# noegroup/aggforce

Hardware: AMD Instinct MI355X
Metric: frames/sec through project_forces (Gram+solve), 1e6x4096-atom traj, 1/2/4/8 GPU (higher is better)
Workload: dtype f64

## Files before the change

aggforce_amd/csrc/aggf_gram.hip:

```cpp
#include <stdlib.h>

#include "aggf_common.h"
#include "aggf_routing.h"

#include <type_traits>

namespace aggf {

constexpr int TILE = 128;
constexpr int ROW_ELEMS = TILE * 3;
constexpr int ROW_PAD = 16;
constexpr int ROW_STRIDE = ROW_ELEMS + ROW_PAD;

template <typename T>
struct GramCfg;
template <>
struct GramCfg<double> {
  static constexpr int KB = 4;
};
template <>
struct GramCfg<float> {
  static constexpr int KB = 8;
};

// ... 269 lines not shown
  if (AHEAD > 1 && n_it > 1) issue_stage(1);
  if (AHEAD > 1 && n_it > 1 && ragged_seq != 1) {
    if constexpr (EDGE) wait_vmcnt_dyn<8>(n_act); else wait_vmcnt<PPW>();
  } else {
    wait_vmcnt<0>();
  }
  asm volatile("s_waitcnt lgkmcnt(0)" ::: "memory");
  __builtin_amdgcn_s_barrier();
  asm volatile("" ::: "memory");

#ifdef AGGF_GRAM_PROF
  uint64_t prof_issue = 0, prof_compute = 0, prof_sync = 0;
#endif
  for (int it = 0; it < n_it; ++it) {
    AGGF_PROF_T(p0);
    constexpr int GROUPS = 3 * KB / 4;
    constexpr bool SPREAD = SPREAD_DMA;
    const bool issue_now = (ABL == 0 || ABL >= 3) && it + AHEAD < n_it;
    if (issue_now) {
      if (SPREAD) prep_stage(it + AHEAD); else issue_stage(it + AHEAD);
    }
    const TS* pa = smem + (((ABL == 1 || ABL == 2) ? it % 2 : it % NBUF)) * BUF_ELEMS;
    AGGF_PROF_T(p1);
    T aL[ES > 0 ? ES : 1][4], bL[ES > 0 ? ES : 1][NACC];
    (void)aL;
    (void)bL;
#pragma unroll
    for (int kk = 0; kk < KB / 4; ++kk) {
#pragma unroll
      for (int d = 0; d < 3; ++d) {
        constexpr int ESG = EARLY_SYNC ? ES : 0;
        const int g = kk * 3 + d;
        T a[4], bb[NACC];
        if (ESG > 0 && g == GROUPS - ESG) {
#pragma unroll
          for (int h = 0; h < (ESG > 0 ? ESG : 1); ++h) {
            const int kh = (GROUPS - ESG + h) / 3, dh = (GROUPS - ESG + h) % 3;
#pragma unroll
            for (int m = 0; m < 4; ++m) aL[h][m] = (T)pa[offA + kh * KKS + 48 * m + dh];
#pragma unroll
            for (int n = 0; n < NACC; ++n) bL[h][n] = (T)pa[offB + kh * KKS + 48 * n + dh];
          }
        }
        if (ESG > 0 && g >= GROUPS - ESG) {
#pragma unroll
          for (int m = 0; m < 4; ++m) a[m] = aL[g - (GROUPS - ESG)][m];
#pragma unroll
          for (int n = 0; n < NACC; ++n) bb[n] = bL[g - (GROUPS - ESG)][n];
        } else {
#pragma unroll
          for (int m = 0; m < 4; ++m) a[m] = (T)pa[offA + kk * KKS + 48 * m + d];
#pragma unroll
          for (int n = 0; n < NACC; ++n) bb[n] = (T)pa[offB + kk * KKS + 48 * n + d];
        }
        constexpr bool DMA_AFTER = ES_DMA_AFTER && ESG > 0;
        if (SPREAD && issue_now && !(DMA_AFTER && g == GROUPS - ESG)) {
#pragma unroll
          for (int q = 0; q < PPW; ++q)
            if (dma_piece_group(GROUPS, PPW, q) == g) issue_piece(it + AHEAD, q);
        }
        if (ESG > 0 && g == GROUPS - ESG) {
          constexpr int ISSUED = dma_pieces_upto(GROUPS, PPW, GROUPS - ESG - (DMA_AFTER ? 1 : 0));
          static_assert(ISSUED >= 0 && ISSUED <= PPW, "pieces issued by the barrier group");
          if (AHEAD > 1 && it + 2 < n_it && it + 2 != ragged_seq) {
            if constexpr (EDGE) wait_vmcnt_dyn<8>(n_act_early); else wait_vmcnt<ISSUED>();
          } else {
            wait_vmcnt<0>();
          }
          asm volatile("s_waitcnt lgkmcnt(0)" ::: "memory");
          __builtin_amdgcn_s_barrier();
          asm volatile("" ::: "memory");
          if (DMA_AFTER && SPREAD && issue_now) {
#pragma unroll
            for (int q = 0; q < PPW; ++q)
              if (dma_piece_group(GROUPS, PPW, q) == g) issue_piece(it + AHEAD, q);
          }
        }
#pragma unroll
        for (int m = 0; m < 4; ++m)
#pragma unroll
          for (int n = 0; n < NACC; ++n) acc[m][n] = M::mma(a[m], bb[n], acc[m][n]);
      }
    }
    AGGF_PROF_T(p2);
    if (ABL != 2 && !EARLY_SYNC) {
      if (AHEAD > 1 && it + 2 < n_it && it + 2 != ragged_seq) {
        if constexpr (EDGE) wait_vmcnt_dyn<8>(n_act); else wait_vmcnt<PPW>();
      } else {
        wait_vmcnt<0>();
      }
      asm volatile("s_waitcnt lgkmcnt(0)" ::: "memory");
      __builtin_amdgcn_s_barrier();
      asm volatile("" ::: "memory");
    }
#ifdef AGGF_GRAM_PROF
    const uint64_t p3 = __builtin_readcyclecounter();
    prof_issue += p1 - p0;
    prof_compute += p2 - p1;
    prof_sync += p3 - p2;
#endif
  }
#ifdef AGGF_GRAM_PROF
  if (lane == 0) {
    atomicAdd(&aggf_gram_prof[0], (unsigned long long)prof_issue);
    atomicAdd(&aggf_gram_prof[1], (unsigned long long)prof_compute);
    atomicAdd(&aggf_gram_prof[2], (unsigned long long)prof_sync);
    atomicAdd(&aggf_gram_prof[3], (unsigned long long)n_it);
  }
#endif

  T* slab = slabs + ((int64_t)tile_lin * ksplit + ks) * (TILE * TILE);
#pragma unroll
  for (int m = 0; m < 4; ++m)
#pragma unroll
    for (int n = 0; n < NACC; ++n)
#pragma unroll
      for (int r = 0; r < 4; ++r) {
        const int row = wm * 64 + m * 16 + M::row(lane, r);
        const int col = wn * WCOLS + n * 16 + (lane & 15);
        slab[row * TILE + col] = acc[m][n][r];
      }
}

__global__ __launch_bounds__(256) void build_tile_table_kernel(int32_t nt1, int32_t* __restrict__ table,
                                                              int32_t first_tile = 0) {
  __shared__ int wave_count[4];
  const int lane = threadIdx.x & 63, wave = threadIdx.x >> 6;
  const int64_t nsb = (nt1 + 7) / 8, n_super = nsb * (nsb + 1) / 2;
  int64_t base = 0;
  for (int64_t b0 = 0; b0 < n_super; b0 += 4) {
    const int64_t sb = b0 + wave;
    bool keep = false;
    int ti = 0, tj = 0;
    if (sb < n_super) {
      const double w = 2.0 * (double)nsb + 1.0;
      int64_t si = (int64_t)((w - sqrt(w * w - 8.0 * (double)sb)) * 0.5);
      if (si < 0) si = 0;
      if (si >= nsb) si = nsb - 1;
      while (si > 0 && si * nsb - si * (si - 1) / 2 > sb) --si;
      while (si + 1 < nsb && (si + 1) * nsb - (si + 1) * si / 2 <= sb) ++si;
      const int64_t sj = si + (sb - (si * nsb - si * (si - 1) / 2));
      ti = (int)si * 8 + (lane >> 3);
      tj = (int)sj * 8 + (lane & 7);
      keep = ti < nt1 && tj < nt1 && tj >= ti && tj >= first_tile;
    }
    const unsigned long long mask = __ballot(keep);
    if (lane == 0) wave_count[wave] = __popcll(mask);
    __syncthreads();
    int64_t off = base;
    for (int w2 = 0; w2 < wave; ++w2) off += wave_count[w2];
    if (keep) table[off + __popcll(mask & ((1ull << lane) - 1ull))] = (ti << 16) | tj;
    base += wave_count[0] + wave_count[1] + wave_count[2] + wave_count[3];
    __syncthreads();
  }
}

template <typename T>
__global__ __launch_bounds__(256) void gram_reduce_kernel(const T* __restrict__ slabs,
                                                          int32_t nt1, int32_t ksplit,
                                                          int32_t n_red, int accumulate,
                                                          double* __restrict__ G, int32_t first_tile = 0) {
  AGGF_GATED_BODY_BEGIN
  int tile = blockIdx.x;
  const int tile_lin = tile;
  int ti = 0;
  {
    int rowlen = nt1;
    while (tile >= rowlen) {
      tile -= rowlen;
      --rowlen;
      ++ti;
    }
  }
  const int tj = ti + tile;
  if (tj < first_tile) return;
  const T* base = slabs + (int64_t)tile_lin * ksplit * (TILE * TILE);
  const int r0 = blockIdx.y * 8;
  for (int e = threadIdx.x; e < 8 * TILE; e += blockDim.x) {
    const int row = r0 + e / TILE, col = e % TILE;
    double s = 0.0;
    for (int ks = 0; ks < ksplit; ++ks)
      s += (double)base[(int64_t)ks * (TILE * TILE) + row * TILE + col];
    const int gi = ti * TILE + row, gj = tj * TILE + col;
    if (gi < n_red && gj < n_red) {
      if (ti != tj || gj >= gi) {
        double* p = G + (int64_t)gi * n_red + gj;
        *p = accumulate ? *p + s : s;
      }
      if (ti != tj || gj > gi) {
        double* p = G + (int64_t)gj * n_red + gi;
        *p = accumulate ? *p + s : s;
      }
    }
  }
  AGGF_GATED_BODY_END
}

constexpr int SM_MAXVEC = 8;
constexpr int SM_FAST_MEMBERS = 4;

template <typename TIn>
static size_t small_raw_bytes(int32_t N, int kbs) { return (size_t)round_up((int64_t)kbs * 3 * N * sizeof(TIn), 16) + 16; }

template <typename TIn, typename TC, int NV, int KBS, int NWV, int W, int C>
__global__ __launch_bounds__(64 * NWV, NWV == 4 ? 3 : 4) void gram_small_kernel(
    const TIn* __restrict__ F, int64_t T, int32_t N, const int32_t* __restrict__ grp_ptr,
    const int32_t* __restrict__ grp_atoms, int32_t n_red, int64_t frames_per_split, int32_t raw_bytes,
    TC* __restrict__ slabs) {
  using M = Mfma<TC>;
  using acc_t = typename M::acc_t;
  constexpr int SM_THREADS = 64 * NWV;
  constexpr int RE = 3 * W, RS = RE + ROW_PAD;
  constexpr int WT = W > TILE ? W : TILE;
  constexpr int SM_ENT = KBS * RE / SM_THREADS;
  constexpr int SM_MAXBLK = C;
  static_assert(KBS * RE % SM_THREADS == 0 && KBS >= 4 && (KBS * W == 8 * TILE || (KBS == 4 && W > 2 * TILE) || (KBS == 8 && W == 2 * TILE)), "entry split");
  typedef float __attribute__((ext_vector_type(4))) v16_t;
  typedef float __attribute__((ext_vector_type(4), aligned(4))) v16g_t;
  extern __shared__ __attribute__((aligned(16))) char smem_raw[];
  TC* panel = reinterpret_cast<TC*>(smem_raw);
  TIn* raw = reinterpret_cast<TIn*>(smem_raw + KBS * RS * sizeof(TC));
  int32_t* atoms_s = reinterpret_cast<int32_t*>(smem_raw + KBS * RS * sizeof(TC) + raw_bytes);
  int32_t* ptr_s = atoms_s + N;
  unsigned short* memb_s = reinterpret_cast<unsigned short*>(smem_raw + KBS * RS * sizeof(TC) + raw_bytes +
                                                             (((int64_t)N + WT + 1) * 4 + 15) / 16 * 16);
  const int tid = threadIdx.x, lane = tid & 63;
  const int wave = __builtin_amdgcn_readfirstlane(tid >> 6);
  (void)frames_per_split;
  const int64_t n_stage_all = (T + KBS - 1) / KBS;
  const int n_it = blockIdx.x < n_stage_all ? (int)((n_stage_all - 1 - blockIdx.x) / gridDim.x + 1) : 0;
  const int64_t t_end = T;
  auto stage_t0 = [&](int k) { return ((int64_t)blockIdx.x + (int64_t)k * gridDim.x) * KBS; };
  const int64_t row_in = (int64_t)N * 3;
  for (int a = tid; a < N; a += SM_THREADS) atoms_s[a] = grp_atoms ? grp_atoms[a] : a;
  for (int g = tid; g <= WT; g += SM_THREADS) ptr_s[g] = g <= n_red ? (grp_ptr ? grp_ptr[g] : g) : (grp_ptr ? grp_ptr[n_red] : n_red);
  const int zero_idx = (raw_bytes - 16) / (int)sizeof(TIn);
  if (tid < 16 / (int)sizeof(TIn)) raw[zero_idx + tid] = (TIn)0;
  __syncthreads();
  bool big_groups = false;
  bool pair_groups = true;
  for (int g = 0; g < n_red; ++g) {
    big_groups |= ptr_s[g + 1] - ptr_s[g] > SM_FAST_MEMBERS;
    pair_groups &= ptr_s[g + 1] - ptr_s[g] <= 2;
  }
  for (int c = tid; c < RE; c += SM_THREADS) {
    const int g = c / 3, d = c - 3 * g;
#pragma unroll
    for (int j = 0; j < SM_FAST_MEMBERS; ++j)
      memb_s[c * 4 + j] = (ptr_s[g] + j < ptr_s[g + 1]) ? (unsigned short)(3 * atoms_s[ptr_s[g] + j] + d) : (unsigned short)0xFFFF;
  }

  const int n_vec = raw_bytes / 16 - 1;
  v16_t hold[NV];
  auto fetch = [&](int s) {
    const int64_t t0 = stage_t0(s);
    const int64_t valid = (t_end - t0 < KBS ? t_end - t0 : KBS) * row_in * (int64_t)sizeof(TIn);
    const char* src = reinterpret_cast<const char*>(F + t0 * row_in);
    if (valid >= (int64_t)n_vec * 16) {
      const unsigned voff = (unsigned)tid * 16u;
      if (gridDim.y == 1) {
#pragma unroll
        for (int i = 0; i < NV; ++i) {
          const int v = tid + SM_THREADS * i;
          const char* base_i = src + (int64_t)i * (SM_THREADS * 16);
          v16_t x = {0.f, 0.f, 0.f, 0.f};
          if (v < n_vec) x = __builtin_nontemporal_load(reinterpret_cast<const v16g_t*>(base_i + voff));
          hold[i] = x;
        }
      } else {
#pragma unroll
        for (int i = 0; i < NV; ++i) {
          const int v = tid + SM_THREADS * i;
          const char* base_i = src + (int64_t)i * (SM_THREADS * 16);
          v16_t x = {0.f, 0.f, 0.f, 0.f};
          if (v < n_vec) x = *reinterpret_cast<const v16g_t*>(base_i + voff);
          hold[i] = x;
        }
      }
    } else {
#pragma unroll
      for (int i = 0; i < NV; ++i) {
        const int v = tid + SM_THREADS * i;
        v16_t x = {0.f, 0.f, 0.f, 0.f};
        if (v < n_vec) {
          const int64_t off = (int64_t)v * 16;
          if (off + 16 <= valid) {
            x = *reinterpret_cast<const v16g_t*>(src + off);
          } else if (off < valid) {
            TIn tmp[16 / sizeof(TIn)];
#pragma unroll
            for (int k = 0; k < (int)(16 / sizeof(TIn)); ++k)
              tmp[k] = off + (k + 1) * (int64_t)sizeof(TIn) <= valid ? reinterpret_cast<const TIn*>(src + off)[k] : (TIn)0;
            x = *reinterpret_cast<v16_t*>(tmp);
          }
        }
        hold[i] = x;
      }
    }
  };
  auto park = [&]() {
#pragma unroll
    for (int i = 0; i < NV; ++i) {
      const int v = tid + SM_THREADS * i;
      if (v < n_vec) reinterpret_cast<v16_t*>(raw)[v] = hold[i];
    }
  };
// ... 68 lines not shown
      panel[r * RS + c] = sum[i];
    }
  };

  const int nb = (n_red + 15) / 16;
  const int n_blocks_all = nb * (nb + 1) / 2;
  const int per_part = (n_blocks_all + (int)gridDim.y - 1) / (int)gridDim.y;
  const int first_block = (int)blockIdx.y * per_part;
  const int n_blocks = n_blocks_all - first_block < per_part ? n_blocks_all - first_block : per_part;
  const bool mfma_wave = wave * C < n_blocks;
  int b_i[SM_MAXBLK], b_j[SM_MAXBLK];
  bool b_real[SM_MAXBLK];
#pragma unroll
  for (int k = 0; k < SM_MAXBLK; ++k) {
    int q = wave * C + k, bi = 0, rowlen = nb;
    b_real[k] = q < n_blocks;
    q = b_real[k] ? q + first_block : 0;
    while (q >= rowlen) {
      q -= rowlen;
      --rowlen;
      ++bi;
    }
    b_i[k] = bi;
    b_j[k] = bi + q;
  }
  acc_t acc[SM_MAXBLK];
#pragma unroll
  for (int k = 0; k < SM_MAXBLK; ++k) acc[k] = acc_zero<TC>();
  const int off = (lane >> 4) * RS + 3 * (lane & 15);

  {
    const unsigned h = ((unsigned)blockIdx.x * 2654435761u) >> 25;
    for (unsigned i = 0; i < h; ++i) __builtin_amdgcn_s_sleep(1);
  }
#ifdef AGGF_SMALL_PROF
  uint64_t pf[7] = {0, 0, 0, 0, 0, 0, 0};
#endif
  if (n_it > 0) fetch(0);
  for (int s = 0; s < n_it; ++s) {
    AGGF_SP_T(q0);
    AGGF_SP_T(q1);
    park();
    AGGF_SP_T(q2);
    __syncthreads();
    AGGF_SP_T(q3);
    if (s + 1 < n_it && (AGGF_SMALL_ABL != 2 || s == 0)) fetch(s + 1);
    AGGF_SP_T(q3b);
    if (AGGF_SMALL_ABL != 3 || s == 0) reduce_groups();
    AGGF_SP_T(q4);
    __syncthreads();
    AGGF_SP_T(q5);
    if (AGGF_SMALL_ABL != 1 && mfma_wave) {
      if constexpr (NWV == 16) {
        constexpr int NPROD = (KBS / 4) * 3 * C;
        auto addr_a = [&](int i) { return off + (i / (3 * C)) * 4 * RS + 48 * b_i[i % C] + (i / C) % 3; };
        auto addr_b = [&](int i) { return off + (i / (3 * C)) * 4 * RS + 48 * b_j[i % C] + (i / C) % 3; };
        TC oa[2], ob[2];
        oa[0] = panel[addr_a(0)];
        ob[0] = panel[addr_b(0)];
#pragma unroll
        for (int i = 0; i < NPROD; ++i) {
          if (i + 1 < NPROD) {
            oa[(i + 1) & 1] = panel[addr_a(i + 1)];
            ob[(i + 1) & 1] = panel[addr_b(i + 1)];
          }
          __builtin_amdgcn_sched_barrier(0);
          acc[i % C] = M::mma(oa[i & 1], ob[i & 1], acc[i % C]);
          __builtin_amdgcn_sched_barrier(0);
        }
      } else {
#pragma unroll
        for (int kk = 0; kk < KBS / 4; ++kk)
#pragma unroll
          for (int d = 0; d < 3; ++d) {
#pragma unroll
            for (int k = 0; k < C; ++k) {
              const TC a = panel[off + kk * 4 * RS + 48 * b_i[k] + d];
              const TC b = panel[off + kk * 4 * RS + 48 * b_j[k] + d];
              acc[k] = M::mma(a, b, acc[k]);
            }
            __builtin_amdgcn_sched_barrier(0);
          }
      }
    }
#ifdef AGGF_SMALL_PROF
    const uint64_t q6 = __builtin_readcyclecounter();
    pf[0] += q1 - q0;
    pf[1] += q2 - q1;
    pf[2] += q3 - q2;
    pf[3] += q4 - q3b;
    pf[6] += q3b - q3;
    pf[4] += q5 - q4;
    pf[5] += q6 - q5;
#endif
  }
#ifdef AGGF_SMALL_PROF
  if (lane == 0) {
    for (int i = 0; i < 7; ++i) atomicAdd(&aggf_small_prof[i], (unsigned long long)pf[i]);
    atomicAdd(&aggf_small_prof[7], (unsigned long long)n_it);
    atomicAdd(&aggf_small_prof[8], 1ull);
  }
#endif
  TC* slab = slabs + ((int64_t)blockIdx.x * gridDim.y + blockIdx.y) * (WT * WT);
#pragma unroll
  for (int k = 0; k < SM_MAXBLK; ++k)
    if (b_real[k]) {
#pragma unroll
      for (int r = 0; r < 4; ++r) slab[(b_i[k] * 16 + M::row(lane, r)) * WT + b_j[k] * 16 + (lane & 15)] = acc[k][r];
    }
}

template <typename T, int WT>
__global__ __launch_bounds__(2 * WT > 1024 ? 1024 : 2 * WT) void gram_reduce_small_kernel(const T* __restrict__ slabs, int32_t ksplit,
                                                                                      int32_t n_red, int accumulate,
                                                                                      double* __restrict__ G, int32_t parts) {
  constexpr int HALVES = 2 * WT > 1024 ? 1 : 2;
  __shared__ double part_sum[HALVES][WT];
  AGGF_GATED_BODY_BEGIN
  const int row = blockIdx.x, col = threadIdx.x & (WT - 1), half = threadIdx.x / WT;
  int owner = 0;
  if (parts > 1 && col >= row) {
    const int nb = (n_red + 15) / 16, bi = row >> 4, bj = col >> 4;
    const int n_blocks = nb * (nb + 1) / 2, per_part = (n_blocks + parts - 1) / parts;
    owner = (bi * nb - bi * (bi - 1) / 2 + (bj - bi)) / per_part;
  }
  double s = 0.0;
  for (int ks = half; ks < ksplit; ks += HALVES) s += (double)slabs[(((int64_t)ks * parts + owner) * WT + row) * WT + col];
  part_sum[half][col] = s;
  __syncthreads();
  if (half == 0 && row < n_red && col < n_red && col >= row) {
    double tot = part_sum[0][col];
    if (HALVES == 2) tot += part_sum[HALVES - 1][col];
    double* p = G + (int64_t)row * n_red + col;
    *p = accumulate ? *p + tot : tot;
    if (col > row) {
      double* q = G + (int64_t)col * n_red + row;
      *q = accumulate ? *q + tot : tot;
    }
  }
  AGGF_GATED_BODY_END
}

enum GramStaging { STAGE_DMA8 = 3, STAGE_SMALL = 4 };

struct GramPlan {
  int32_t n_pad, nt1, n_tiles;
  int32_t first_tile = 0;
  int staging;
  int32_t n_entries;
  bool direct;
  int ksplit;
  bool edge = false;
  bool straddle = false;
  bool wide256 = false;
  int parts = 1;
  int64_t frames_per_split;
  int64_t chunk_frames;
  size_t slab_bytes, pack_bytes;
};

static int choose_ksplit(int n_tiles, int64_t frames, int kb, int slots, int64_t max_splits, int stage_rows = 0) {
  if (stage_rows <= 0) stage_rows = kb;
  int64_t hi = ceil_div(frames, (int64_t)stage_rows * 8);
  if (hi < 1) hi = 1;
  if (hi > max_splits) hi = max_splits;
  if (hi > 1024) hi = 1024;
  static const char* force_k = getenv("AGGF_GRAM_KSPLIT");
  if (force_k && atoi(force_k) > 0) return (int)(atoi(force_k) < hi ? atoi(force_k) : hi);
  const double us_per_frame = 0.64 * 4.0 / kb;
  const double fixed_frames = 48.0;
  const double slab_us = 2.0 * TILE * TILE * (kb == 4 ? 8 : 4) / 2.0e6;
  double best_cost = 1e300;
  int64_t best = 1;
  for (int64_t k = 1; k <= hi; ++k) {
    const int64_t blocks = k * n_tiles;
    const double rounds = (double)ceil_div(blocks, slots);
    const double fpb = (double)round_up(ceil_div(frames, k), stage_rows);
    const double cost = rounds * (fpb + fixed_frames) * us_per_frame + blocks * slab_us;
    if (cost < best_cost * (1.0 - 1e-6)) {
      best_cost = cost;
      best = k;
    }
  }
  return (int)best;
}

static size_t dtype_size(int dt) { return dt == AGGF_F64 ? 8 : 4; }
static size_t table_bytes(const GramPlan& p) { return (size_t)round_up((int64_t)p.n_tiles * 8, 256); }

static int make_plan(int64_t T, int32_t N, int32_t n_red, int in_dtype, int compute_dtype,
                     bool has_groups, bool aligned, size_t ws_bytes, bool query, GramPlan* p, int32_t first_col = 0,
                     bool tiles_only = false) {
  p->n_pad = (int32_t)round_up(n_red, TILE);
  p->nt1 = p->n_pad / TILE;
  p->n_tiles = p->nt1 * (p->nt1 + 1) / 2;
  p->edge = N % TILE != 0;
  const bool widen = in_dtype == AGGF_F32 && compute_dtype == AGGF_F64;
  const bool rows16 = ((int64_t)3 * N * (int64_t)dtype_size(in_dtype)) % 16 == 0;
  p->straddle = p->edge && !rows16 && !tiles_only && first_col == 0 && T >= 2;
  p->direct = !has_groups && (in_dtype == compute_dtype || (widen && !tiles_only)) && aligned &&
              (!p->edge || (!tiles_only && (rows16 || p->straddle)));
  if (!p->direct) p->straddle = false;
  p->staging = STAGE_DMA8;
  static const char* no_small = getenv("AGGF_GRAM_NO_SMALL");
  const size_t raw_small = (size_t)round_up((int64_t)8 * 3 * N * (int64_t)dtype_size(in_dtype), 16);
  const size_t raw_wide = (size_t)round_up((int64_t)4 * 3 * N * (int64_t)dtype_size(in_dtype), 16);
  const bool wide_fits = first_col == 0 && raw_wide <= (size_t)5 * 64 * 16 * 16;
  const char* route = getenv("AGGF_GRAM_ROUTE");
  const bool force_stream = route && route[0] == 's', force_tile = route && route[0] == 't';
  const bool f64p = compute_dtype == AGGF_F64;
  const int edge3_max = widen ? routing::stream_edge3_max_cols_widen : routing::stream_edge3_max_cols;
  const int edge4_max = widen ? routing::stream_edge4_max_cols_widen
                              : (f64p ? routing::stream_edge4_max_cols_f64 : routing::stream_edge4_max_cols_f32);
  const bool wide = wide_fits && (p->nt1 == 2 || (force_stream && p->nt1 <= 4) ||
                                  (p->nt1 == 3 && (!p->direct || (p->edge && n_red <= edge3_max))) ||
                                  (p->nt1 == 4 && !p->direct && n_red <= (f64p ? routing::stream_pack4_max_cols_f64 : routing::stream_pack4_max_cols_f32)) ||
                                  (p->nt1 == 4 && p->direct && p->edge && n_red <= edge4_max));
  p->parts = 1;
  p->wide256 = wide_fits && p->nt1 == 1 && n_red > routing::wide256_min_cols && !has_groups;
  if (((p->nt1 == 1 && raw_small <= (size_t)SM_MAXVEC * 64 * 8 * 16) || wide || p->wide256) && !no_small && !force_tile && !tiles_only && N < 21000 && aligned) {
    p->staging = STAGE_SMALL;
    p->n_entries = 1;
    p->direct = true;
    p->chunk_frames = T;
    p->pack_bytes = 0;
    const int nb16 = (n_red + 15) / 16, n_blocks = nb16 * (nb16 + 1) / 2;
    if (p->nt1 > 2) p->parts = (int)ceil_div((int64_t)n_blocks, compute_dtype == AGGF_F32 ? 192 : 144);
    int64_t nwg = (int64_t)(p->nt1 >= 2 || p->wide256 ? 1 : 2) * device_cu_count() / p->parts;
    if (nwg < 1) nwg = 1;
    const int64_t n_stage_all = ceil_div(T, 8);
    if (nwg > n_stage_all) nwg = n_stage_all;
    const int64_t edge = p->nt1 > 2 ? 4 * TILE : (p->wide256 ? 2 * TILE : p->n_pad);
    const size_t slab1s = (size_t)p->parts * edge * edge * dtype_size(compute_dtype);
    if (!query) {
      if (ws_bytes < table_bytes(*p) + slab1s + 512) return fail(AGGF_ERR_WORKSPACE, "gram workspace too small");
      const int64_t max_splits = (int64_t)((ws_bytes - table_bytes(*p) - 512) / slab1s);
      if (nwg > max_splits) nwg = max_splits;
    }
    p->frames_per_split = 0;
    p->ksplit = (int)nwg;
    p->slab_bytes = (size_t)p->ksplit * slab1s;
    return AGGF_OK;
  }
  p->n_entries = p->n_tiles;
  p->first_tile = 0;
  if (first_col >= TILE && p->direct) {
    p->first_tile = first_col / TILE;
    if (p->first_tile >= p->nt1) p->first_tile = p->nt1 - 1;
    p->n_entries = p->n_tiles - p->first_tile * (p->first_tile + 1) / 2;
  }
  const int kb = compute_dtype == AGGF_F64 ? GramCfg<double>::KB : GramCfg<float>::KB;
  const int stage_rows = p->direct && widen ? GramCfg<float>::KB : kb;
  const size_t cs = dtype_size(compute_dtype);
  const int slots = 2 * device_cu_count();
  const size_t slab1 = (size_t)p->n_tiles * TILE * TILE * cs;
  const size_t row_bytes = (size_t)p->n_pad * 3 * cs;
  if (query) {
    p->chunk_frames = T;
    if (!p->direct) {
      size_t free_b = 0, total_b = 0;
      size_t cap_b = (size_t)16 << 30;
      if (hipMemGetInfo(&free_b, &total_b) == hipSuccess && free_b / 4 < cap_b) cap_b = free_b / 4;
      if (cap_b < ((size_t)1 << 28)) cap_b = (size_t)1 << 28;
      int64_t cf = (int64_t)(cap_b / row_bytes);
      if (cf < 256) cf = 256;
      if (cf > T) cf = T;
      p->chunk_frames = cf > 0 ? cf : 1;
    }
    p->ksplit = choose_ksplit(p->n_entries, p->chunk_frames, kb, slots, 1 << 20, stage_rows);
    p->slab_bytes = slab1 * p->ksplit;
    p->pack_bytes = p->direct ? 0 : round_up((int64_t)(p->chunk_frames * row_bytes), 256);
    return AGGF_OK;
  }
  p->pack_bytes = 0;
  p->chunk_frames = T;
  if (ws_bytes < table_bytes(*p) + 1024) return fail(AGGF_ERR_WORKSPACE, "gram workspace too small");
  ws_bytes -= table_bytes(*p);
  size_t avail = ws_bytes;
  if (!p->direct) {
    size_t slab_budget = slab1 * (size_t)choose_ksplit(p->n_entries, T, kb, slots, 1 << 20) + 1024;
    if (slab_budget > ws_bytes / 2) slab_budget = ws_bytes / 2;
    int64_t cf = (int64_t)((ws_bytes - slab_budget) / row_bytes);
    if (cf > T) cf = T;
    if (cf < 1) return fail(AGGF_ERR_WORKSPACE, "gram workspace too small for one packed frame");
    p->chunk_frames = cf;
    p->pack_bytes = (size_t)round_up((int64_t)(cf * row_bytes), 256);
    avail = ws_bytes - p->pack_bytes;
  }
  avail = avail > 512 ? avail - 512 : 0;
  const int64_t max_splits = (int64_t)(avail / slab1);
  if (max_splits < 1) return fail(AGGF_ERR_WORKSPACE, "gram workspace too small for one slab set");
  p->ksplit = choose_ksplit(p->n_entries, p->chunk_frames, kb, slots, max_splits, stage_rows);
  p->slab_bytes = slab1 * p->ksplit;
  return AGGF_OK;
}

template <typename TIn>
__global__ __launch_bounds__(256) void gram_tail_row_kernel(const TIn* __restrict__ row, int32_t n_red, double* __restrict__ G) {
  const int i = blockIdx.y * 16 + threadIdx.y, j = blockIdx.x * 16 + threadIdx.x;
  if (i >= n_red || j >= n_red) return;
  double s = 0.0;
#pragma unroll
  for (int d = 0; d < 3; ++d) s += (double)row[3 * i + d] * (double)row[3 * j + d];
  G[(int64_t)i * n_red + j] += s;
}

template <typename T, bool EDGE = false, typename TS = T>
static int launch_gram(const TS* X, int64_t rows, int64_t ld, const GramPlan& p, T* slabs,
                       int32_t* tile_table, double* G, int32_t n_red, int accumulate, hipStream_t stream,
                       bool straddle = false) {
  constexpr int KB = GramCfg<TS>::KB;
  const int ksplit = p.ksplit;
  int64_t fps = round_up(ceil_div(rows, ksplit), KB);
  if (fps < KB) fps = KB;
  const int64_t nblocks = (int64_t)ksplit * p.n_tiles;
  if (nblocks > 0x7fffffffLL) return fail(AGGF_ERR_ARG, "gram grid too large");
  const size_t lds3 = (size_t)3 * 2 * dma_panel_elems<TS>() * sizeof(TS);
  static thread_local PerDeviceOnce attr_once;
  bool& attr_done = *attr_once.flag();
  if (!attr_done) {
    AGGF_HIP_OK(hipFuncSetAttribute((const void*)gram_tile_dma_kernel<T, 0, 3, 2, 8, true, 1, true, false, EDGE, TS>,
                                    hipFuncAttributeMaxDynamicSharedMemorySize, (int)lds3));
    attr_done = true;
  }
  AGGF_LAUNCH(build_tile_table_kernel, dim3(1), dim3(256), 0, stream, p.nt1, tile_table, p.first_tile);
  AGGF_LAUNCH_OK();
  const int64_t nblk = (int64_t)ksplit * p.n_entries;
  AGGF_LAUNCH((gram_tile_dma_kernel<T, 0, 3, 2, 8, true, 1, true, false, EDGE, TS>), dim3((unsigned)round_up(nblk, 512)),
                     dim3(512), lds3, stream, X, rows, ld, p.nt1, p.n_entries, ksplit, tile_table, fps, slabs,
                     (const TS*)nullptr, (int64_t)0, 0, (int32_t)(EDGE ? ld : 0), (int32_t)(straddle ? 1 : 0));
  AGGF_LAUNCH_OK();
  AGGF_LAUNCH_GATED(1024, (gram_reduce_kernel<T>), dim3(p.n_tiles, TILE / 8), dim3(256), 0, stream,
                     slabs, p.nt1, ksplit, n_red, accumulate, G, p.first_tile);
  AGGF_LAUNCH_OK();
  return AGGF_OK;
}

struct PackPipe {
  hipStream_t side = nullptr;
  hipEvent_t packed[2] = {nullptr, nullptr}, consumed[2] = {nullptr, nullptr};
  bool ok = false, tried = false;
};
static PackPipe* pack_pipe() {
  static thread_local PackPipe pipes[64];
  int dev = 0;
  if (hipGetDevice(&dev) != hipSuccess || dev < 0 || dev >= 64) return nullptr;
  PackPipe& pp = pipes[dev];
  if (!pp.tried) {
    pp.tried = true;
    bool ok = hipStreamCreateWithFlags(&pp.side, hipStreamNonBlocking) == hipSuccess;
    for (int k = 0; k < 2 && ok; ++k)
      ok = hipEventCreateWithFlags(&pp.packed[k], hipEventDisableTiming) == hipSuccess &&
           hipEventCreateWithFlags(&pp.consumed[k], hipEventDisableTiming) == hipSuccess;
    pp.ok = ok;
  }
  return pp.ok ? &pp : nullptr;
}

template <typename TIn, typename TC>
static int gram_typed(const void* Fv, int64_t T, int32_t N, const int32_t* grp_ptr,
                      const int32_t* grp_atoms, int32_t n_red, double* G, int accumulate,
                      const GramPlan& p, char* ws, hipStream_t stream) {
  int32_t* tile_table = reinterpret_cast<int32_t*>(ws);
  ws += table_bytes(p);
  TC* slabs = reinterpret_cast<TC*>(ws);
  if (p.staging == STAGE_SMALL) {
    constexpr int threads = 512;
    int width = n_red <= 32 ? 32 : (n_red <= 64 ? 64 : TILE);
    while (width < TILE && small_raw_bytes<TIn>(N, 8 * TILE / width) / 16 - 1 > (size_t)SM_MAXVEC * threads) width *= 2;
    if (p.nt1 == 2 || p.wide256) width = 2 * TILE;
    if (p.nt1 > 2) width = 4 * TILE;
    int kbs = width > 2 * TILE ? 4 : 8 * TILE / width;
    if (width == 2 * TILE && small_raw_bytes<TIn>(N, 8) / 16 - 1 <= (size_t)5 * 1024 &&
        ((n_red + 15) / 16) * ((n_red + 15) / 16 + 1) / 2 <= 5 * 16)
      kbs = 8;
    const int wt = width > TILE ? width : TILE;
    const int n_thr = width > TILE ? 1024 : threads;
    const size_t raw_bytes = small_raw_bytes<TIn>(N, kbs);
    const size_t lds = (size_t)kbs * (3 * width + ROW_PAD) * sizeof(TC) + raw_bytes +
                       (size_t)round_up(((int64_t)N + wt + 1) * 4, 16) + (size_t)3 * width * 4 * sizeof(unsigned short);
    const int nv = (int)ceil_div((int64_t)(raw_bytes / 16 - 1), n_thr);
    if (nv > SM_MAXVEC || (width > TILE && nv > 5)) return fail(AGGF_ERR_ARG, "aggf_gram: small-system kernel: frame too large");
    const int nb16 = (n_red + 15) / 16, n_blocks = nb16 * (nb16 + 1) / 2;
    const int per_part = (int)ceil_div((int64_t)n_blocks, p.parts);
    const int per_wave = (int)ceil_div((int64_t)per_part, width > TILE ? 16 : 8);
#define AGGF_SMALL(NVC, KBC, NWC, WC, CC)                                                                            \
  do {                                                                                                               \
    if (lds > 65536) {                                                                                               \
      static thread_local PerDeviceOnce attr_once;                                                                   \
      bool& attr_done = *attr_once.flag();                                                                           \
      if (!attr_done) {                                                                                              \
        AGGF_HIP_OK(hipFuncSetAttribute((const void*)gram_small_kernel<TIn, TC, NVC, KBC, NWC, WC, CC>,              \
                                        hipFuncAttributeMaxDynamicSharedMemorySize, 160 * 1024 - 1024));             \
        attr_done = true;                                                                                            \
      }                                                                                                              \
    }                                                                                                                \
    AGGF_LAUNCH((gram_small_kernel<TIn, TC, NVC, KBC, NWC, WC, CC>), dim3((unsigned)p.ksplit, (unsigned)p.parts), \
                       dim3(64 * NWC), lds, stream, reinterpret_cast<const TIn*>(Fv), T, N, grp_ptr, grp_atoms,      \
                       n_red, p.frames_per_split, (int32_t)raw_bytes, slabs);                                        \
  } while (0)
#define AGGF_SMALL_NV(KBC, WC, CC)                                                                                   \
  do {                                                                                                               \
    if (nv <= 3) AGGF_SMALL(3, KBC, 8, WC, CC);                                                                      \
    else if (nv <= 5) AGGF_SMALL(5, KBC, 8, WC, CC);                                                                 \
    else AGGF_SMALL(8, KBC, 8, WC, CC);                                                                              \
  } while (0)
#define AGGF_SMALL_WIDE(WC, CC)                                                                                      \
  do {                                                                                                               \
    if (nv <= 3) AGGF_SMALL(3, 4, 16, WC, CC);                                                                       \
    else AGGF_SMALL(5, 4, 16, WC, CC);                                                                               \
  } while (0)
#define AGGF_SMALL_WIDE8(CC)                                                                                         \
  do {                                                                                                               \
    if (nv <= 3) AGGF_SMALL(3, 8, 16, 2 * TILE, CC);                                                                 \
    else AGGF_SMALL(5, 8, 16, 2 * TILE, CC);                                                                         \
  } while (0)
    if (width == 32) AGGF_SMALL_NV(32, 32, 1);
    else if (width == 64 && per_wave <= 1) AGGF_SMALL_NV(16, 64, 1);
    else if (width == 64) AGGF_SMALL_NV(16, 64, 2);
    else if (width == TILE && per_wave <= 2) AGGF_SMALL_NV(8, TILE, 2);
    else if (width == TILE && per_wave == 3) AGGF_SMALL_NV(8, TILE, 3);
    else if (width == TILE && per_wave == 4) AGGF_SMALL_NV(8, TILE, 4);
    else if (width == TILE) AGGF_SMALL_NV(8, TILE, 5);
    else if (width == 2 * TILE && kbs == 8 && per_wave <= 3) AGGF_SMALL_WIDE8(3);
    else if (width == 2 * TILE && kbs == 8 && per_wave == 4) AGGF_SMALL_WIDE8(4);
    else if (width == 2 * TILE && kbs == 8) AGGF_SMALL_WIDE8(5);
    else if (width == 2 * TILE && per_wave <= 3) AGGF_SMALL_WIDE(2 * TILE, 3);
    else if (width == 2 * TILE && per_wave == 4) AGGF_SMALL_WIDE(2 * TILE, 4);
    else if (width == 2 * TILE && per_wave == 5) AGGF_SMALL_WIDE(2 * TILE, 5);
    else if (width == 2 * TILE && per_wave == 6) AGGF_SMALL_WIDE(2 * TILE, 6);
    else if (width == 2 * TILE && per_wave == 7) AGGF_SMALL_WIDE(2 * TILE, 7);
    else if (width == 2 * TILE && per_wave == 8) AGGF_SMALL_WIDE(2 * TILE, 8);
    else if (width == 2 * TILE) AGGF_SMALL_WIDE(2 * TILE, 9);
    else if (per_wave <= 6) {
      if constexpr (std::is_same<TC, float>::value) {
        AGGF_SMALL_WIDE(4 * TILE, 7);
      } else {
        if (per_wave <= 5) AGGF_SMALL_WIDE(4 * TILE, 5);
        else AGGF_SMALL_WIDE(4 * TILE, 6);
      }
    }
    else if (per_wave == 7) AGGF_SMALL_WIDE(4 * TILE, 7);
    else if (per_wave == 8) AGGF_SMALL_WIDE(4 * TILE, 8);
    else if (per_wave == 9) AGGF_SMALL_WIDE(4 * TILE, 9);
    else {
      if constexpr (std::is_same<TC, float>::value) {
        if (per_wave == 10) AGGF_SMALL_WIDE(4 * TILE, 10);
        else if (per_wave == 11) AGGF_SMALL_WIDE(4 * TILE, 11);
        else AGGF_SMALL_WIDE(4 * TILE, 12);
      } else {
        return fail(AGGF_ERR_ARG, "aggf_gram: streaming kernel: more than 144 blocks per workgroup with float64 products");
      }
    }
#undef AGGF_SMALL_WIDE
#undef AGGF_SMALL_WIDE8
#undef AGGF_SMALL_NV
#undef AGGF_SMALL
    AGGF_LAUNCH_OK();
    if (width == 4 * TILE)
      AGGF_LAUNCH_GATED(256, (gram_reduce_small_kernel<TC, 4 * TILE>), dim3(4 * TILE), dim3(1024), 0, stream, slabs, p.ksplit,
                         n_red, accumulate, G, p.parts);
    else if (width > TILE)
      AGGF_LAUNCH_GATED(256, (gram_reduce_small_kernel<TC, 2 * TILE>), dim3(2 * TILE), dim3(4 * TILE), 0, stream, slabs, p.ksplit,
// ... 229 lines not shown
```

aggforce_amd/csrc/aggf_routing.h:

```cpp
#pragma once

namespace aggf {
namespace routing {

constexpr int stream_edge3_max_cols = 320;
constexpr int stream_pack4_max_cols_f64 = 400;
constexpr int stream_pack4_max_cols_f32 = 512;
constexpr int stream_edge4_max_cols_f64 = 400;
constexpr int stream_edge4_max_cols_f32 = 512;
constexpr int stream_edge3_max_cols_widen = 352;
constexpr int stream_edge4_max_cols_widen = 424;
constexpr int wide256_min_cols = 112;
constexpr int pack_overlap_min_pad = 1408;

}
}
```

Measured before the change: 1.179 million.

## Add paired-tile macro Gram kernel sharing staged panels across two output tiles

Adds a 1024-thread f64 Gram kernel that computes two adjacent upper-triangular 128x128 tiles per block. It stages up to three distinct column panels per frame chunk in LDS, so shared panels are loaded once for both tiles, and a new macro table pairs the tiles. The aim is to cut global-to-LDS traffic and DMA issue overhead per tile. In exchange it uses larger blocks (one per CU in the slot model), a different ksplit cost model, and a pairing scheme whose leftover handling adds complexity. It is routed for aligned f64 cases with at least 9 column tiles.

```diff
diff --git a/aggforce_amd/csrc/aggf_gram.hip b/aggforce_amd/csrc/aggf_gram.hip
--- a/aggforce_amd/csrc/aggf_gram.hip
+++ b/aggforce_amd/csrc/aggf_gram.hip
@@ -445,6 +445,244 @@
     if (keep) table[off + __popcll(mask & ((1ull << lane) - 1ull))] = (ti << 16) | tj;
     base += wave_count[0] + wave_count[1] + wave_count[2] + wave_count[3];
     __syncthreads();
+  }
+}
+
+template <int NBUF_, int KB_, int AHEAD_, bool BURST_, bool STAGGER_, int PG_ = 3 * KB_ / 4>
+struct MacroForm {
+  static constexpr int NBUF = NBUF_, KB = KB_, AHEAD = AHEAD_, PG = PG_;
+  static constexpr bool BURST = BURST_, STAGGER = STAGGER_;
+};
+constexpr int MACRO_PANELS = 3;
+using MacroShipped = MacroForm<2, 8, 1, false, false, 5>;
+
+template <int NBUF, int KB, int AHEAD, bool BURST, bool STAGGER, int PG>
+__global__ __launch_bounds__(1024, 1) void gram_tile_dma_kernel_x2(
+    const double* __restrict__ X, int64_t n_rows, int64_t ld, int32_t nt1, int32_t n_macro, int32_t ksplit,
+    const int32_t* __restrict__ macro_table, int64_t frames_per_split, double* __restrict__ slabs) {
+  using M = Mfma<double>;
+  constexpr int NW = 16;
+  constexpr int GROUPS = 3 * KB / 4;
+  constexpr int PANEL_ELEMS = KB * ROW_STRIDE;
+  constexpr int BUF_ELEMS = MACRO_PANELS * PANEL_ELEMS;
+  constexpr int PPP = KB * 3;
+  constexpr int PPW = (MACRO_PANELS * PPP + NW - 1) / NW;
+  constexpr int NTHREADS = 64 * NW;
+  constexpr int KKS = 4 * ROW_STRIDE;
+  static_assert(KB == 4 || KB == 8, "frames per stage");
+  static_assert(PG >= 1 && PG <= GROUPS, "groups that take a DMA piece");
+  static_assert(AHEAD >= 1 && AHEAD <= NBUF - 1 - ((STAGGER && !BURST) ? 1 : 0), "ring depth");
+  static_assert(AHEAD >= 2 || (!BURST && !STAGGER && PG < GROUPS), "pieces behind the barrier need AHEAD >= 2");
+
+  extern __shared__ __attribute__((aligned(16))) char smem_raw[];
+  double* smem = reinterpret_cast<double*>(smem_raw);
+
+  const int tid = threadIdx.x;
+  const int lane = tid & 63;
+  const int wave = __builtin_amdgcn_readfirstlane(tid >> 6);
+  const int half = wave >> 3;
+  const int wm = (wave & 7) >> 2, wn = wave & 3;
+
+  const int b = blockIdx.x;
+  const int v = (((b >> 3) >> 5) * 8 + (b & 7)) * 32 + ((b >> 3) & 31);
+  if (v >= ksplit * n_macro) return;
+  const int ks = v / n_macro;
+  const int ent = v - ks * n_macro;
+  const int tA = macro_table[2 * ent], tB = macro_table[2 * ent + 1];
+  const bool lone = tB < 0;
+  const int tiA = tA >> 16, tjA = tA & 0xffff;
+  const int tiB = lone ? tiA : tB >> 16, tjB = lone ? tjA : tB & 0xffff;
+  int p0 = tiA, p1 = -1, p2 = -1, np = 1;
+  auto add_panel = [&](int c) {
+    if (c != p0 && c != p1 && c != p2) {
+      if (np == 1) p1 = c; else p2 = c;
+      ++np;
+    }
+  };
+  add_panel(tjA);
+  add_panel(tiB);
+  add_panel(tjB);
+  auto slot_of = [&](int c) { return c == p0 ? 0 : (c == p1 ? 1 : 2); };
+  const int ti = half ? tiB : tiA, tj = half ? tjB : tjA;
+  const int tile_lin = ti * nt1 - ti * (ti - 1) / 2 + (tj - ti);
+
+  const int64_t t_begin = (int64_t)ks * frames_per_split;
+  int64_t t_end = t_begin + frames_per_split;
+  if (t_end > n_rows) t_end = n_rows;
+  const int n_it = t_begin < t_end ? (int)((t_end - t_begin + KB - 1) / KB) : 0;
+  const int last_rows = n_it > 0 ? (int)(t_end - t_begin - (int64_t)(n_it - 1) * KB) : KB;
+
+  int64_t g_off[PPW];
+  int l_off[PPW], p_row[PPW];
+  bool p_ok[PPW];
+  int n_act = 0, n_act_last = 0;
+#pragma unroll
+  for (int q = 0; q < PPW; ++q) {
+    const int p = wave + NW * q;
+    const int panel = p / PPP;
+    const int unit = (p - panel * PPP) / 3;
+    const int cp = p % 3;
+    const int pcol = panel == 0 ? p0 : (panel == 1 ? p1 : p2);
+    p_ok[q] = panel < np;
+    p_row[q] = unit;
+    g_off[q] = (int64_t)unit * ld + (int64_t)pcol * ROW_ELEMS + cp * 128 + lane * 2;
+    l_off[q] = panel * PANEL_ELEMS + unit * ROW_STRIDE + cp * 128;
+    n_act += p_ok[q] ? 1 : 0;
+    n_act_last += (p_ok[q] && unit < last_rows) ? 1 : 0;
+  }
+
+  const int skew = n_it > 16 ? ((tiA + (tjA >> 1)) & 7) : 0;
+  auto stage_of = [&](int seq) { const int s = seq + skew; return s >= n_it ? s - n_it : s; };
+  const bool ragged = n_it > 0 && last_rows != KB;
+  const int ragged_seq = ragged ? (n_it - 1 - skew + (n_it - 1 - skew < 0 ? n_it : 0)) : -1;
+  auto issued_upto = [&](int seq) {
+    const int s = seq < n_it - 1 ? seq : n_it - 1;
+    return (s + 1) * n_act - ((ragged_seq >= 0 && s >= ragged_seq) ? n_act - n_act_last : 0);
+  };
+  int n_iss = 0;
+  auto prep_stage = [&](int seq) {
+    if (seq == ragged_seq) {
+      double* lbase = smem + (seq % NBUF) * BUF_ELEMS;
+      const int nz = KB - last_rows;
+      for (int e = tid; e < MACRO_PANELS * nz * ROW_ELEMS; e += NTHREADS) {
+        const int panel = e / (nz * ROW_ELEMS);
+        const int rem = e - panel * nz * ROW_ELEMS;
+        const int r = last_rows + rem / ROW_ELEMS, c = rem % ROW_ELEMS;
+        lbase[panel * PANEL_ELEMS + r * ROW_STRIDE + c] = 0;
+      }
+    }
+  };
+  auto issue_piece = [&](int seq, int q) {
+    const int st = stage_of(seq);
+    const int64_t t0 = t_begin + (int64_t)st * KB;
+    if (seq < n_it && p_ok[q] && p_row[q] < (st == n_it - 1 ? last_rows : KB)) {
+      __builtin_amdgcn_global_load_lds(
+          (const __attribute__((address_space(1))) void*)(X + t0 * ld + g_off[q]),
+          (__attribute__((address_space(3))) void*)(smem + (seq % NBUF) * BUF_ELEMS + l_off[q]), 16, 0, 0);
+      ++n_iss;
+    }
+  };
+  auto wait_landed = [&](int seq) {
+    wait_vmcnt_dyn<8>(n_iss - issued_upto(seq));
+    asm volatile("s_waitcnt lgkmcnt(0)" ::: "memory");
+  };
+
+  f64x4 acc[4][2];
+#pragma unroll
+  for (int m = 0; m < 4; ++m)
+#pragma unroll
+    for (int n = 0; n < 2; ++n) acc[m][n] = acc_zero<double>();
+  const int offA = slot_of(ti) * PANEL_ELEMS + (lane >> 4) * ROW_STRIDE + 3 * (wm * 64 + (lane & 15));
+  const int offB = slot_of(tj) * PANEL_ELEMS + (lane >> 4) * ROW_STRIDE + 3 * (wn * 32 + (lane & 15));
+
+#pragma unroll
+  for (int s = 0; s < AHEAD; ++s)
+    if (s < n_it) {
+      prep_stage(s);
+#pragma unroll
+      for (int q = 0; q < PPW; ++q) issue_piece(s, q);
+    }
+  wait_landed(0);
+  __builtin_amdgcn_s_barrier();
+  asm volatile("" ::: "memory");
+
+  const int bar_g = (STAGGER && half) ? 0 : GROUPS - 1;
+  const bool prep_early = !BURST && bar_g != 0;
+  for (int it = 0; it < n_it; ++it) {
+    const bool issue_now = it + AHEAD < n_it;
+    if (issue_now && prep_early) prep_stage(it + AHEAD);
+    const double* pa = smem + (it % NBUF) * BUF_ELEMS;
+#pragma unroll
+    for (int kk = 0; kk < KB / 4; ++kk) {
+#pragma unroll
+      for (int d = 0; d < 3; ++d) {
+        const int g = kk * 3 + d;
+        double a[4], bb[2];
+#pragma unroll
+        for (int m = 0; m < 4; ++m) a[m] = pa[offA + kk * KKS + 48 * m + d];
+#pragma unroll
+        for (int n = 0; n < 2; ++n) bb[n] = pa[offB + kk * KKS + 48 * n + d];
+        if (g == bar_g) {
+          wait_landed(it + 1);
+          __builtin_amdgcn_s_barrier();
+          asm volatile("" ::: "memory");
+          if (issue_now) {
+            if (!prep_early) prep_stage(it + AHEAD);
+#pragma unroll
+            for (int q = 0; q < PPW; ++q)
+              if (BURST || q * PG / PPW == g) issue_piece(it + AHEAD, q);
+          }
+        } else if (!BURST && issue_now) {
+#pragma unroll
+          for (int q = 0; q < PPW; ++q)
+            if (q * PG / PPW == g) issue_piece(it + AHEAD, q);
+        }
+#pragma unroll
+        for (int m = 0; m < 4; ++m)
+#pragma unroll
+          for (int n = 0; n < 2; ++n) acc[m][n] = M::mma(a[m], bb[n], acc[m][n]);
+      }
+    }
+  }
+
+  if (half && lone) return;
+  double* slab = slabs + ((int64_t)tile_lin * ksplit + ks) * (TILE * TILE);
+#pragma unroll
+  for (int m = 0; m < 4; ++m)
+#pragma unroll
+    for (int n = 0; n < 2; ++n)
+#pragma unroll
+      for (int r = 0; r < 4; ++r) {
+        const int row = wm * 64 + m * 16 + M::row(lane, r);
+        const int col = wn * 32 + n * 16 + (lane & 15);
+        slab[row * TILE + col] = acc[m][n][r];
+      }
+}
+
+__host__ __device__ static inline int macro_leftovers(int nt1) { return (nt1 + 1) / 2; }
+__host__ __device__ static inline int macro_count(int nt1) {
+  const int n_left = macro_leftovers(nt1);
+  return (nt1 * (nt1 + 1) / 2 - n_left) / 2 + (n_left + 1) / 2;
+}
+__global__ __launch_bounds__(256) void build_macro_table_kernel(int32_t nt1, int32_t* __restrict__ table) {
+  __shared__ int wave_count[4];
+  const int lane = threadIdx.x & 63, wave = threadIdx.x >> 6;
+  const int64_t nsb = (nt1 + 7) / 8, n_super = nsb * (nsb + 1) / 2;
+  int64_t base = 0;
+  for (int64_t b0 = 0; b0 < n_super; b0 += 4) {
+    const int64_t sb = b0 + wave;
+    bool keep = false;
+    int ti = 0, tj = 0;
+    if (sb < n_super) {
+      const double w = 2.0 * (double)nsb + 1.0;
+      int64_t si = (int64_t)((w - sqrt(w * w - 8.0 * (double)sb)) * 0.5);
+      if (si < 0) si = 0;
+      if (si >= nsb) si = nsb - 1;
+      while (si > 0 && si * nsb - si * (si - 1) / 2 > sb) --si;
+      while (si + 1 < nsb && (si + 1) * nsb - (si + 1) * si / 2 <= sb) ++si;
+      const int64_t sj = si + (sb - (si * nsb - si * (si - 1) / 2));
+      ti = (int)si * 8 + (lane >> 3);
+      tj = (int)sj * 8 + (lane & 7);
+      keep = ti < nt1 && tj < nt1 && tj >= ti && ((nt1 - tj) & 1) == 0;
+    }
+    const unsigned long long mask = __ballot(keep);
+    if (lane == 0) wave_count[wave] = __popcll(mask);
+    __syncthreads();
+    int64_t off = base;
+    for (int w2 = 0; w2 < wave; ++w2) off += wave_count[w2];
+    if (keep) {
+      const int64_t k = off + __popcll(mask & ((1ull << lane) - 1ull));
+      table[2 * k] = (ti << 16) | tj;
+      table[2 * k + 1] = (ti << 16) | (tj + 1);
+    }
+    base += wave_count[0] + wave_count[1] + wave_count[2] + wave_count[3];
+    __syncthreads();
+  }
+  const int n_left = macro_leftovers(nt1), first = (nt1 - 1) & 1;
+  for (int k = threadIdx.x; 2 * k < n_left; k += blockDim.x) {
+    const int a = first + 4 * k, c = a + 2;
+    table[2 * (base + k)] = (a << 16) | a;
+    table[2 * (base + k) + 1] = 2 * k + 1 < n_left ? ((c << 16) | c) : -1;
   }
 }
 
@@ -819,6 +1057,7 @@
   int ksplit;
   bool edge = false;
   bool straddle = false;
+  bool macro = false;
   bool wide256 = false;
   int parts = 1;
   int64_t frames_per_split;
@@ -826,7 +1065,8 @@
   size_t slab_bytes, pack_bytes;
 };
 
-static int choose_ksplit(int n_tiles, int64_t frames, int kb, int slots, int64_t max_splits, int stage_rows = 0) {
+static int choose_ksplit(int n_tiles, int64_t frames, int kb, int slots, int64_t max_splits, int stage_rows = 0,
+                         int tiles_per_entry = 1) {
   if (stage_rows <= 0) stage_rows = kb;
   int64_t hi = ceil_div(frames, (int64_t)stage_rows * 8);
   if (hi < 1) hi = 1;
@@ -843,7 +1083,7 @@
     const int64_t blocks = k * n_tiles;
     const double rounds = (double)ceil_div(blocks, slots);
     const double fpb = (double)round_up(ceil_div(frames, k), stage_rows);
-    const double cost = rounds * (fpb + fixed_frames) * us_per_frame + blocks * slab_us;
+    const double cost = rounds * (fpb + fixed_frames) * us_per_frame + blocks * tiles_per_entry * slab_us;
     if (cost < best_cost * (1.0 - 1e-6)) {
       best_cost = cost;
       best = k;
@@ -874,7 +1114,8 @@
   const size_t raw_wide = (size_t)round_up((int64_t)4 * 3 * N * (int64_t)dtype_size(in_dtype), 16);
   const bool wide_fits = first_col == 0 && raw_wide <= (size_t)5 * 64 * 16 * 16;
   const char* route = getenv("AGGF_GRAM_ROUTE");
-  const bool force_stream = route && route[0] == 's', force_tile = route && route[0] == 't';
+  const bool force_stream = route && route[0] == 's' && route[1] == 't', force_tile = route && route[0] == 't';
+  const bool force_single = route && route[0] == 's' && route[1] == 'i', force_macro = route && route[0] == 'm';
   const bool f64p = compute_dtype == AGGF_F64;
   const int edge3_max = widen ? routing::stream_edge3_max_cols_widen : routing::stream_edge3_max_cols;
   const int edge4_max = widen ? routing::stream_edge4_max_cols_widen
@@ -916,10 +1157,14 @@
     if (p->first_tile >= p->nt1) p->first_tile = p->nt1 - 1;
     p->n_entries = p->n_tiles - p->first_tile * (p->first_tile + 1) / 2;
   }
+  p->macro = p->direct && !p->edge && in_dtype == AGGF_F64 && compute_dtype == AGGF_F64 && first_col == 0 &&
+             !tiles_only && (p->nt1 >= routing::macro_min_tiles || force_macro) && !force_single;
+  if (p->macro) p->n_entries = macro_count(p->nt1);
+  const int tpe = p->macro ? 2 : 1;
   const int kb = compute_dtype == AGGF_F64 ? GramCfg<double>::KB : GramCfg<float>::KB;
-  const int stage_rows = p->direct && widen ? GramCfg<float>::KB : kb;
+  const int stage_rows = p->direct && widen ? GramCfg<float>::KB : (p->macro ? MacroShipped::KB : kb);
   const size_t cs = dtype_size(compute_dtype);
-  const int slots = 2 * device_cu_count();
+  const int slots = (p->macro ? 1 : 2) * device_cu_count();
   const size_t slab1 = (size_t)p->n_tiles * TILE * TILE * cs;
   const size_t row_bytes = (size_t)p->n_pad * 3 * cs;
   if (query) {
@@ -934,7 +1179,7 @@
       if (cf > T) cf = T;
       p->chunk_frames = cf > 0 ? cf : 1;
     }
-    p->ksplit = choose_ksplit(p->n_entries, p->chunk_frames, kb, slots, 1 << 20, stage_rows);
+    p->ksplit = choose_ksplit(p->n_entries, p->chunk_frames, kb, slots, 1 << 20, stage_rows, tpe);
     p->slab_bytes = slab1 * p->ksplit;
     p->pack_bytes = p->direct ? 0 : round_up((int64_t)(p->chunk_frames * row_bytes), 256);
     return AGGF_OK;
@@ -957,7 +1202,7 @@
   avail = avail > 512 ? avail - 512 : 0;
   const int64_t max_splits = (int64_t)(avail / slab1);
   if (max_splits < 1) return fail(AGGF_ERR_WORKSPACE, "gram workspace too small for one slab set");
-  p->ksplit = choose_ksplit(p->n_entries, p->chunk_frames, kb, slots, max_splits, stage_rows);
+  p->ksplit = choose_ksplit(p->n_entries, p->chunk_frames, kb, slots, max_splits, stage_rows, tpe);
   p->slab_bytes = slab1 * p->ksplit;
   return AGGF_OK;
 }
@@ -972,10 +1217,43 @@
   G[(int64_t)i * n_red + j] += s;
 }
 
+template <typename FORM>
+static int launch_gram_macro(const double* X, int64_t rows, int64_t ld, const GramPlan& p, double* slabs,
+                             int32_t* tile_table, double* G, int32_t n_red, int accumulate, hipStream_t stream) {
+  constexpr int KB = FORM::KB;
+  const int ksplit = p.ksplit;
+  int64_t fps = round_up(ceil_div(rows, ksplit), KB);
+  if (fps < KB) fps = KB;
+  const int n_macro = macro_count(p.nt1);
+  const int64_t nblk = (int64_t)ksplit * n_macro;
+  if (round_up(nblk, 256) > 0x7fffffffLL) return fail(AGGF_ERR_ARG, "gram grid too large");
+  const size_t lds = (size_t)FORM::NBUF * MACRO_PANELS * KB * ROW_STRIDE * sizeof(double);
+  auto kernel = gram_tile_dma_kernel_x2<FORM::NBUF, KB, FORM::AHEAD, FORM::BURST, FORM::STAGGER, FORM::PG>;
+  static thread_local PerDeviceOnce attr_once;
+  bool& attr_done = *attr_once.flag();
+  if (!attr_done) {
+    AGGF_HIP_OK(hipFuncSetAttribute((const void*)kernel, hipFuncAttributeMaxDynamicSharedMemorySize, (int)lds));
+    attr_done = true;
+  }
+  AGGF_LAUNCH(build_macro_table_kernel, dim3(1), dim3(256), 0, stream, p.nt1, tile_table);
+  AGGF_LAUNCH_OK();
+  AGGF_LAUNCH((gram_tile_dma_kernel_x2<FORM::NBUF, KB, FORM::AHEAD, FORM::BURST, FORM::STAGGER, FORM::PG>),
+              dim3((unsigned)round_up(nblk, 256)), dim3(1024), lds, stream, X, rows, ld, p.nt1, n_macro, ksplit, tile_table,
+              fps, slabs);
+  AGGF_LAUNCH_OK();
+  AGGF_LAUNCH_GATED(1024, (gram_reduce_kernel<double>), dim3(p.n_tiles, TILE / 8), dim3(256), 0, stream,
+                     slabs, p.nt1, ksplit, n_red, accumulate, G, 0);
+  AGGF_LAUNCH_OK();
+  return AGGF_OK;
+}
+
 template <typename T, bool EDGE = false, typename TS = T>
 static int launch_gram(const TS* X, int64_t rows, int64_t ld, const GramPlan& p, T* slabs,
                        int32_t* tile_table, double* G, int32_t n_red, int accumulate, hipStream_t stream,
                        bool straddle = false) {
+  if constexpr (std::is_same<T, double>::value && std::is_same<TS, double>::value && !EDGE) {
+    if (p.macro) return launch_gram_macro<MacroShipped>(X, rows, ld, p, slabs, tile_table, G, n_red, accumulate, stream);
+  }
   constexpr int KB = GramCfg<TS>::KB;
   const int ksplit = p.ksplit;
   int64_t fps = round_up(ceil_div(rows, ksplit), KB);
diff --git a/aggforce_amd/csrc/aggf_routing.h b/aggforce_amd/csrc/aggf_routing.h
--- a/aggforce_amd/csrc/aggf_routing.h
+++ b/aggforce_amd/csrc/aggf_routing.h
@@ -12,6 +12,7 @@
 constexpr int stream_edge4_max_cols_widen = 424;
 constexpr int wide256_min_cols = 112;
 constexpr int pack_overlap_min_pad = 1408;
+constexpr int macro_min_tiles = 9;
 
 }
 }
```

Result: faster. 1.241 million (median of 6 runs) (+5.2%).
